# EmreAdabag/osqp

Hardware: AMD Instinct MI355X
Metric: ADMM iters/sec (single QP) (higher is better)
Workload: dtype f64; 1 GPU; config2 random sparse QP n=10000 m=20000 nnzA=200000 nnzPtriu=59985, one step = osqp_update_rho(0.1) + cold-started osqp_solve; adaptive_rho_interval=100, status=solved, graph_launches=4775, resident_gave_up=0, resident_slow_waits=0, parallelism=replicas x1 (a single QP does not shard)

## Files before the change

osqp_amd/csrc/engine.hip:

```cpp
#include <hip/hip_runtime.h>
#include <cstdio>
#include <new>
#include <cstdlib>
#include <cstring>
#include <cmath>
#include <vector>
#include <map>
#include <algorithm>
#include <mutex>
#include <condition_variable>
#include <thread>
#include <atomic>
#include <chrono>
#include "../../include/osqp_amd_engine.h"

#define TB 256
#define MAX_CHUNK 2048
#define LONG_ROW 512
#define HUGE_ROW 8192
#define MAX_PARTS 1024
#define MAX_HUGE_FOLD 4
#define INF_BOUND 1e26

#define HIPCHK(call)                                                            \
// ... 9 lines not shown
struct RowBlk { int r0, r1, k0, k1; };
#define IS_LONG(b) ((b).r1 - (b).r0 == 1 && (b).k1 - (b).k0 >= LONG_ROW)
struct __attribute__((aligned(32))) G4 { double r, w, s, m; };

struct DevMat {
  int nrows, nblk;
  int nstream;
  int nwave;
  const int    *rowptr;
  const int    *col;
  const unsigned short *col16;
  const double *val;
  const int    *split;
  const RowBlk *blk;
};

#define DENSE_MAX 128
struct DenseBlk { int c0, b, off, pitch; };
struct DenseP {
  int nblk;
  const DenseBlk *blk;
  const double *val;
};

struct State {
  int    run;
  int    done;
  int    stalled;
  int    neg_curv;
  int    iters[2];
  int    neg_curv_seen;
  int    iters_last;
  int    iters_max;
  int    iters_min;
  int    forced;
  long long iters_total;
  long long admm_done;
  double rz[2];
  double tol2;
  double gam[2], alp[2];
  int    hist_r;
  long long admm_target;
  unsigned res_epoch;
  int    res_fail;
  int    res_pipe_off;
  int    res_chk_fail;
  int    res_dbg[4];
  int    res_slow;
  int    res_slow_max;
  int    res_repub;
  int    res_slow_hist[4];
  unsigned res_slow_xcc;
  int    res_slow_last[4];
};

struct Params {
  double sigma, alpha, eps_rel, eps_abs, cinv;
  int    pcg_max_iter, use_cvec, has_scaling, pad0;
  double ex_theta;
  int    ex_h0, ex_h1;
  int    no_restart;
};

struct Ctx {
  int n, m;
  DevMat A, M;
  DevMat Mk;
  DenseP dP;
  int nh, hrow[MAX_HUGE_FOLD];
  const double *hcol;
  int gridA, gridM;
  double *xy, *z, *zt, *va, *vb, *q, *l, *u, *rho, *rhoinv, *minv, *pdiag;
  double *r, *zz, *kp, *pt0, *pt1, *dxy, *dy, *cvec;
  double *init_r, *init_z;
  double *vx, *vold;
  double *pdir, *ut;
  G4     *g4;
  int     init_stride;
  int     fin_wave_rows;
  double *vd;
  int     plain_rhs;
  const int *plain_skip;
  const unsigned short *u0map;
  double *u0pos;
  int     nelim;
  const int *erow, *ecol, *epos;
  double *rhoe, *ecoef, *edinv, *xte;
  double *D, *Dinv, *E, *Einv;
  double *part_rz, *part_rr, *part_bb, *part_pkp, *part_s0, *part_s1, *part_s2, *part_gam, *part_del;
  const double *fin_rr;
  int fin_cnt;
  double *scal;
  double *part_h;
  State  *st;
  const Params *prm;
#ifdef OSQP_AMD_TIMELINE
  unsigned long long *tl;
#endif
};

#ifdef OSQP_AMD_TIMELINE
#define TL_CAP (1 << 20)
#define TL_MARK(c, id) do { if (blockIdx.x == 0 && threadIdx.x == 0) { const unsigned long long k_ = atomicAdd((c).tl, 1ull); \
    if (k_ < TL_CAP - 2) (c).tl[1 + k_] = ((unsigned long long)(id) << 56) | (wall_clock64() & 0x00FFFFFFFFFFFFFFull); } } while (0)
#else
#define TL_MARK(c, id) do { } while (0)
#endif

enum {
  SC_PRI_U, SC_PRI_S, SC_Z_U, SC_Z_S, SC_AX_U, SC_AX_S,
  SC_DUA_U, SC_DUA_S, SC_Q_U, SC_Q_S, SC_ATY_U, SC_ATY_S, SC_PX_U, SC_PX_S,
  SC_DYN_U, SC_DYN_S, SC_DXN_U, SC_DXN_S,
  SC_ATDY_U, SC_ATDY_S, SC_PDX_U, SC_PDX_S, SC_ADX_VIOL,
  SC_OBJ, SC_DYLHS, SC_QDX,
  SC_COUNT
};
#define SCI(x) ((x) * 16)

template <int CTRL>
__device__ __forceinline__ double dpp_move(double v) {
  int lo = __double2loint(v), hi = __double2hiint(v);
  lo = __builtin_amdgcn_mov_dpp(lo, CTRL, 0xF, 0xF, true); hi = __builtin_amdgcn_mov_dpp(hi, CTRL, 0xF, 0xF, true);
  return __hiloint2double(hi, lo);
}
__device__ __forceinline__ double lane_value(double v, int lane) {
  return __hiloint2double(__builtin_amdgcn_readlane(__double2hiint(v), lane), __builtin_amdgcn_readlane(__double2loint(v), lane));
}
__device__ __forceinline__ double wave_sum(double v) {
  v += dpp_move<0xB1>(v); v += dpp_move<0x4E>(v); v += dpp_move<0x141>(v); v += dpp_move<0x140>(v);
  return (lane_value(v, 0) + lane_value(v, 16)) + (lane_value(v, 32) + lane_value(v, 48));
}

__device__ __forceinline__ double block_sum(double v, double *red) {
  v = wave_sum(v);
  const int lane = threadIdx.x & 63, w = threadIdx.x >> 6;
  __syncthreads();
  if (lane == 0) red[w] = v;
// ... 218 lines not shown
    const double rj = gone ? 0.0 : bj - prm.sigma * c.vx[j] - sA;
    const double zj = c.minv[j] * rj;
    c.init_r[(size_t)j * c.init_stride] = rj;
    c.init_z[j] = zj;
    if (c.u0pos) c.u0pos[c.u0map[j]] = zj;
    prz += rj * zj; prr += rj * rj; pbb += bj * bj;
  };
  for (int bi = blockIdx.x; bi < Mm.nstream; bi += gridDim.x) {
    const RowBlk b = Mm.blk[bi];
    stage_products<2>(Mm, b, c.vx, c.vb, lprod, lprod + MAX_CHUNK);
    __syncthreads();
    const int RL = lanes_for(b.r1 - b.r0), rg = threadIdx.x / RL, rlane = threadIdx.x % RL;
    for (int j = b.r0 + rg; j < b.r1; j += TB / RL) {
      const int a0 = Mm.rowptr[j] - b.k0, a1 = Mm.rowptr[j + 1] - b.k0;
      const double sA = row_sum_par(lprod, a0, a1, rlane, RL);
      const double sB = row_sum_par(lprod + MAX_CHUNK, a0, a1, rlane, RL);
      if (rlane == 0) row_start(j, sA, sB);
    }
    __syncthreads();
  }
  for (int bi = Mm.nstream + blockIdx.x * (TB / 64) + (threadIdx.x >> 6); bi < Mm.nblk; bi += gridDim.x * (TB / 64)) {
    const RowBlk lb = Mm.blk[bi];
    const int lane = threadIdx.x & 63;
    if (c.vd) {
      const double acc = wave_row_dot(Mm, lb.k0, lb.k1, [&](int cc) { return c.vd[cc]; });
      if (lane == 0) row_start(lb.r0, -acc, 0.0);
      continue;
    }
    double a0 = 0.0, a1 = 0.0, b0 = 0.0, b1 = 0.0;
    const bool narrow = Mm.col16 != nullptr;
    constexpr int UI = 8;
    for (int k0 = lb.k0 + lane; k0 - lane < lb.k1; k0 += 64 * UI) {
      int cc[UI]; double vv[UI], xa[UI], xb[UI];
#pragma unroll
      for (int q = 0; q < UI; ++q) {
        const int kc = min(k0 + 64 * q, lb.k1 - 1);
        cc[q] = narrow ? (int)Mm.col16[kc] : Mm.col[kc];
        vv[q] = Mm.val[kc];
      }
#pragma unroll
      for (int q = 0; q < UI; ++q) { xa[q] = c.vx[cc[q]]; xb[q] = c.vb[cc[q]]; }
#pragma unroll
      for (int q = 0; q < UI; ++q) if (k0 + 64 * q >= lb.k1) vv[q] = 0.0;
#pragma unroll
      for (int q = 0; q < UI; q += 2) { a0 += vv[q] * xa[q]; b0 += vv[q] * xb[q]; a1 += vv[q + 1] * xa[q + 1]; b1 += vv[q + 1] * xb[q + 1]; }
    }
    const double sA = wave_sum(a0 + a1), sB = wave_sum(b0 + b1);
    if (lane == 0) row_start(lb.r0, sA, sB);
  }
  block_sum3(prz, prr, pbb, red);
  if (threadIdx.x == 0) {
    c.part_rz[blockIdx.x] = prz; c.part_rr[blockIdx.x] = prr; c.part_bb[blockIdx.x] = pbb;
    if (blockIdx.x == 0) {
      st->run = 1; st->done = 0; st->neg_curv = 0; st->iters[0] = 0; st->iters[1] = 0;
      if (st->hist_r < (1 << 20)) st->hist_r += 1;
    }
  }
}

#define EPT (MAX_CHUNK / TB)

struct CgStep { double alpha, beta; bool first, stop, conv, bad; };
__device__ __forceinline__ CgStep cg_step(double rr, double gam, double del, double gam_old, double alp_old,
                                          double tol2, int iters_prev, int neg, const Params &prm, bool bench) {
  CgStep s;
  s.first = gam_old == 0.0;
  s.bad = false;
  if (s.first) { s.beta = 0.0; s.alpha = gam / del; }
  else {
    s.beta = gam / gam_old;
    const double den = del - s.beta * gam / alp_old;
    if (!(den > 0.0) && del > 0.0) {
      if (!prm.no_restart && rr <= 1e8 * tol2) { s.first = true; s.beta = 0.0; s.alpha = gam / del; }
      else { s.alpha = gam / den; s.bad = true; }
    } else s.alpha = gam / den;
  }
  if (bench) { s.beta = 0.5; s.alpha = 1e-3; s.bad = false; }
  s.conv = rr <= tol2;
  s.bad = s.bad || !(s.alpha > 0.0) || !(del > 0.0);
  s.stop = !bench && (s.conv || iters_prev >= prm.pcg_max_iter || neg || s.bad);
  return s;
}
__global__ void __launch_bounds__(TB) k_cg_A(Ctx c, int it, int flags) {
  State *st = c.st;
  TL_MARK(c, 2);
  const bool bench = flags & 4, upd_only = flags & 16, apply_only = flags & 32;
  const bool pre = (flags & 8) || apply_only;
  if (!bench && it >= (flags >> 8) && (it >= st->iters_last || st->stalled) && (!st->run || st->done)) return;
  const int stalled = st->stalled, run = st->run, done = st->done, neg = st->neg_curv;
  const int iters_prev = st->iters[(it + 1) & 1];
  const double tol2_old = st->tol2, gam_old = st->gam[(it + 1) & 1], alp_old = st->alp[(it + 1) & 1];
  const Params prm = *c.prm;
  const bool has_blk = (int)blockIdx.x < c.A.nstream;
  RowBlk b = {0, 0, 0, 0};
  if (has_blk) b = c.A.blk[blockIdx.x];
  const int cnt = b.k1 - b.k0;
  const bool small = has_blk;
  const G4 *gold = c.g4 + (size_t)((it + 1) & 1) * c.n;
  G4 *gnew = c.g4 + (size_t)(it & 1) * c.n;
  int ecol[EPT]; double eval[EPT], g0[EPT], g1[EPT], g2[EPT], g3[EPT];
  int RL = lanes_for(b.r1 - b.r0);
  int rg = threadIdx.x / RL, rlane = threadIdx.x % RL;
  int rp0 = 0, rp1 = 0;
  double prho = 0.0;
  if (small) {
    if (b.r0 + rg < b.r1) { rp0 = c.A.rowptr[b.r0 + rg]; rp1 = c.A.rowptr[b.r0 + rg + 1]; prho = c.rhoe[b.r0 + rg]; }
#pragma unroll
// ... 253 lines not shown
      const double uj = lprod[4 * DENSE_MAX + threadIdx.x], wj = (acc + sigma * uj) + hterm(jrow, false), rj = gc[jrow].r;
      gc[jrow].w = wj; pg += rj * uj; pd += wj * uj; prr += rj * rj;
    }
    __syncthreads();
  }
  block_sum3(pg, pd, prr, red);
  if (threadIdx.x == 0) { c.part_gam[blockIdx.x] = pg; c.part_del[blockIdx.x] = pd; c.part_rr[blockIdx.x] = prr; }
}


__global__ void __launch_bounds__(TB) k_huge_dot(Ctx c, const double *x, int always) {
  if (!always && !c.st->run) return;
  if (!x) {
    const State *st = c.st;
    x = (c.vx != c.va && st->iters[0] == 0 && st->iters[1] == 0) ? c.vx : c.va;
  }
  __shared__ double red[16];
  for (int bi = c.A.nwave; bi < c.A.nblk; ++bi) {
    const RowBlk hb = c.A.blk[bi];
    double s0 = 0.0, s1 = 0.0;
    int k = hb.k0 + blockIdx.x * TB + threadIdx.x;
    const int stride = gridDim.x * TB;
    for (; k + stride < hb.k1; k += 2 * stride) {
      const int c0 = c.A.col[k], c1 = c.A.col[k + stride];
      s0 += c.A.val[k] * x[c0]; s1 += c.A.val[k + stride] * x[c1];
    }
    if (k < hb.k1) s0 += c.A.val[k] * x[c.A.col[k]];
    const double tot = block_sum(s0 + s1, red);
    if (threadIdx.x == 0) c.part_h[(size_t)(bi - c.A.nwave) * gridDim.x + blockIdx.x] = tot;
  }
}
__device__ __forceinline__ double huge_row_sum(const Ctx &c, int bi, double *red) {
  const double *part = c.part_h + (size_t)(bi - c.A.nwave) * c.gridA;
  double s = 0.0;
  for (int i = threadIdx.x; i < c.gridA; i += TB) s += part[i];
  return block_sum(s, red);
}

__device__ __forceinline__ double elim_vb(const Ctx &c, const Params &prm, int i, double rho, double vbn, double x_y) {
  const int y = c.ecol[i];
  if (y < 0) return vbn;
  const double a = c.ecoef[i];
  const double by = (prm.use_cvec ? c.cvec[y] : (prm.sigma * x_y - c.q[y])) + a * vbn;
  return vbn - rho * a * by * c.edinv[i];
}

__global__ void __launch_bounds__(TB) k_admm_finalize(Ctx c) {
  State *st = c.st;
  TL_MARK(c, 4);
  if (!st->run || st->res_fail) return;
  LDS_DECL(1);
  const Params prm = *c.prm;
  double rr[1];
  reduce_parts<1>(c.fin_rr, nullptr, nullptr, c.fin_cnt, red, rr);
  const int iters = st->iters[0] > st->iters[1] ? st->iters[0] : st->iters[1];
  const bool conv = st->done == 1 || rr[0] <= st->tol2;
  const bool force = st->done == 2 || iters >= prm.pcg_max_iter || st->neg_curv;
  if (!conv && !force) {
    if (blockIdx.x == 0 && threadIdx.x == 0) st->stalled = 1;
    return;
  }
  if (blockIdx.x == 0 && threadIdx.x == 0) {
    st->stalled = 0;
    st->admm_done += 1;
    st->iters_last = iters;
    st->iters_total += iters;
    if (iters > st->iters_max) st->iters_max = iters;
    if (iters < st->iters_min) st->iters_min = iters;
    if (!conv) st->forced += 1;
    if (st->neg_curv) st->neg_curv_seen += 1;
  }
  const double alpha = prm.alpha, oma = 1.0 - prm.alpha;
  const int hist = st->hist_r;
  const double th = (hist < prm.ex_h0 ? 0.0 : (hist < prm.ex_h1 ? 0.5 : 1.0)) * prm.ex_theta;
  const bool ex = c.vx != c.va;
  const bool from_start = ex && iters == 0;
  const double *xts = from_start ? c.vx : c.va;
  double *x = c.xy, *y = c.xy + c.n;
  for (int j = blockIdx.x * TB + threadIdx.x; j < c.n; j += gridDim.x * TB) {
    if (c.nelim && c.erow[j] >= 0) continue;
    const double xo = x[j], xt = xts[j];
    const double xn = alpha * xt + oma * xo;
    c.dxy[j] = xn - xo;
    x[j] = xn;
    if (ex) { c.vx[j] = xt + th * (xt - c.vold[j]); c.vold[j] = xt; }
    if (from_start) c.va[j] = xt;
  }
  auto row_update = [&](int i, double zt) {
    const double rho = c.rho[i], rinv = c.rhoinv[i], yo = y[i], zo = c.z[i];
    const int ye = c.nelim ? c.ecol[i] : -1;
    double rz = rho * zt, xny = 0.0;
    if (ye >= 0) {
      const double a = c.ecoef[i], xoy = x[ye];
      const double by = (prm.use_cvec ? c.cvec[ye] : (prm.sigma * xoy - c.q[ye])) + a * (rho * zo - yo);
      const double xty = (by - rho * a * zt) * c.edinv[i];
      rz = c.rhoe[i] * zt;
      zt += a * xty;
      xny = alpha * xty + oma * xoy;
      c.dxy[ye] = xny - xoy; x[ye] = xny; c.xte[i] = xty;
    }
    double v = alpha * zt + oma * zo + rinv * yo;
    v = fmax(v, c.l[i]);
    const double zn = fmin(v, c.u[i]);
    const double dy = rho * (alpha * zt + oma * zo - zn);
    const double yn = yo + dy;
    c.z[i] = zn; y[i] = yn; c.dy[i] = dy; c.zt[i] = zt;
    c.va[c.n + i] = rz;
    if (ex) { c.vx[c.n + i] = rz + th * (rz - c.vold[c.n + i]); c.vold[c.n + i] = rz; }
    c.vb[c.n + i] = ye >= 0 ? elim_vb(c, prm, i, rho, rho * zn - yn, xny) : rho * zn - yn;
  };
// ... 108 lines not shown
    for (int eb = e0; eb < e1; eb += 256) {
      int j[4]; double v[4];
#pragma unroll
      for (int q = 0; q < 4; ++q) {
        const int idx = eb + q * 64 + lane;
        j[q] = -1; v[q] = 0.0;
        if (idx < e1) {
          j[q] = rc.kcj[idx];
          const int ps = rc.kps[idx];
          v[q] = (ps >= 0 ? c.M.val[ps] : 0.0) + (j[q] == i ? sigma : 0.0);
        }
      }
      for (int kc = ka; kc < kb; kc += 64) {
        const bool on = kc + lane < kb;
        const int kk = on ? c.M.col[kc + lane] - c.n : 0;
        const double ai = on ? c.M.val[kc + lane] : 0.0, rk = on ? c.rhoe[kk] : 0.0;
        const int p0 = on ? c.A.rowptr[kk] : 0, p1 = on ? c.A.rowptr[kk + 1] : 0;
        const int cnt = min(64, kb - kc);
        for (int q = 0; q < cnt; ++q) {
          const double a_i = lane_value(ai, q), r = lane_value(rk, q);
          const int s0 = lane_int(p0, q), s1 = lane_int(p1, q);
          for (int ec = s0; ec < s1; ec += 64) {
            const bool eon = ec + lane < s1;
            const int cj = eon ? c.A.col[ec + lane] : -1;
            const double av = eon ? c.A.val[ec + lane] : 0.0;
            const int len = min(64, s1 - ec);
            for (int e = 0; e < len; ++e) {
              const int cjb = lane_int(cj, e);
              const double t = r * (a_i * lane_value(av, e));
#pragma unroll
              for (int q4 = 0; q4 < 4; ++q4) if (j[q4] == cjb) v[q4] += t;
            }
          }
        }
      }
      const bool igone = c.nelim && c.erow[i] >= 0;
#pragma unroll
      for (int q = 0; q < 4; ++q) {
        const int idx = eb + q * 64 + lane;
        if (idx < e1) {
          const bool gone = c.nelim && (igone || c.erow[j[q]] >= 0);
          rc.val[rc.kdst[idx]] = gone ? (j[q] == i ? 1.0 : 0.0) : v[q];
        }
      }
    }
  }
}

template <int E>
__global__ void __launch_bounds__(RES_TB) k_pcg_resident(Ctx c, ResCtx rc) {
  extern __shared__ __attribute__((aligned(16))) double rlds[];
  State *st = c.st;
  TL_MARK(c, 5);
  if (st->stalled || !st->run || st->res_fail) return;
  double *uv = rlds;
  double *seg = uv + rc.npad;
  double *sc = seg + RES_TB + RES_MAXROWS;
  double *sval = sc + 8;
#ifdef OSQP_AMD_TIMELINE
  long long *tls = reinterpret_cast<long long *>(sval + 768);
#define RTL(k) do { if (blockIdx.x == 0 && threadIdx.x == 0 && nx >= 1 && nx <= 64) tls[(nx - 1) * 5 + (k)] = wall_clock64(); } while (0)
  long long *wtl = tls + 5 * 64;
#define WTL(k) do { if (blockIdx.x == 0 && (threadIdx.x & 63) == 0 && (nx == 8 || nx == 1)) wtl[(nx == 1 ? 40 : 0) + (k) * 8 + (threadIdx.x >> 6)] = wall_clock64(); } while (0)
  if (blockIdx.x == 0 && threadIdx.x == 0) wtl[80] = wall_clock64();
#else
#define RTL(k) do { } while (0)
#define WTL(k) do { } while (0)
#endif
  const int g = blockIdx.x, t = threadIdx.x, lane = t & 63, wv = t >> 6;
  const int nwg = rc.nwg, npad = rc.npad;
  const ResWG w = rc.wg[g];
  const Params prm = *c.prm;
  const unsigned ep0 = st->res_epoch;
  const bool sabotage = rc.inject > 0 && g == rc.nwg - 1 && st->admm_done + 1 == rc.inject;
  bool pipe = rc.pipe && !st->res_pipe_off && !prm.no_restart;
  const bool prod = wv != 0;
  const int tt = t - 64;
  double kv[E]; unsigned short kc[E];
#pragma unroll
  for (int k = 0; k < E; ++k) { kv[k] = 0.0; kc[k] = 0; }
  unsigned long long brk = 0ull;
  int slot0 = 0;
  if (prod) {
#pragma unroll
    for (int k = 0; k < E; ++k) {
      const size_t idx = ((size_t)g * E + k) * RES_PT + tt;
      kv[k] = rc.val[idx]; kc[k] = rc.col[idx];
    }
    brk = rc.brk[(size_t)g * RES_PT + tt];
    slot0 = rc.slot0[(size_t)g * RES_PT + tt];
  }
  int sr0 = 0, sr1 = 0;
  int ppos[4];
#pragma unroll
  for (int q = 0; q < 4; ++q) { const int o = lane + 64 * q; ppos[q] = 0; if (o < rc.nwg) { const ResWG wo = rc.wg[o]; ppos[q] = wo.pos + wo.nr; } }
  double rr0 = 0.0, bb = 0.0;
  for (int i = lane; i < c.gridM; i += 64) { rr0 += c.part_rr[i]; bb += c.part_bb[i]; }
  rr0 = wave_sum(rr0); bb = wave_sum(bb);
  const double tol2 = fmax(prm.eps_rel * prm.eps_rel * bb, prm.eps_abs * prm.eps_abs);
  if (rr0 <= tol2) {
    if (g == 0 && t == 0) { st->done = 1; st->tol2 = tol2; }
    return;
  }
  const bool own = wv == 0 && lane < w.nr;
  const int j = w.r0 + lane;
  double r_ = 0, u_ = 0, w_ = 0, p_ = 0, s_ = 0, x_ = 0, mi = 0, x0_ = 0, r0_ = 0;
  double z_ = 0, q_ = 0;
  if (own) {
    r_ = c.init_r[(size_t)j * c.init_stride]; u_ = c.init_z[j]; x_ = c.vx[j]; mi = c.minv[j];
    x0_ = x_; r0_ = r_;
    sr0 = rc.segrow[(size_t)g * (RES_MAXROWS + 1) + lane]; sr1 = rc.segrow[(size_t)g * (RES_MAXROWS + 1) + lane + 1];
  }
  if (t == 0) sc[3] = 0.0;
  __syncthreads();
  int nx = 0;
  unsigned tag = ep0;
  int par = 0;

  auto vec_exchange = [&](double val, bool ride) __attribute__((always_inline)) -> bool {
    double e0 = 0.0, e1 = 0.0, e2 = 0.0;
    ++nx; tag = ep0 + (unsigned)nx; par = (int)(tag & 1u);
    if (sabotage && nx == 3) return false;
    RTL(0);
    const __amdgpu_buffer_rsrc_t rs = res_rsrc(rc.ubuf + (size_t)par * npad, (size_t)npad * 8);
    if (wv == 0) {
      if (lane < w.nr) {
        u32x2 d; d.x = (unsigned)__double2loint(val); d.y = (unsigned)__double2hiint(val);
        __builtin_amdgcn_raw_buffer_store_b64(d, rs, (w.pos + lane) * 8, 0, AUX_SC1);
      }
      if (ride) { e0 = wave_sum(own ? r_ * u_ : 0.0); e1 = wave_sum(own ? w_ * u_ : 0.0); e2 = wave_sum(own ? r_ * r_ : 0.0); }
      if (lane < 3) {
        const double v = lane == 0 ? e0 : (lane == 1 ? e1 : e2);
        u32x2 d; d.x = (unsigned)__double2loint(v); d.y = (unsigned)__double2hiint(v);
        __builtin_amdgcn_raw_buffer_store_b64(d, rs, (w.pos + w.nr + lane) * 8, 0, AUX_SC1);
      }
      asm volatile("s_waitcnt vmcnt(0)" ::: "memory");
      if (lane == 0) __hip_atomic_store(rc.flags + (size_t)g * RES_FSTRIDE, tag, __ATOMIC_RELAXED, __HIP_MEMORY_SCOPE_AGENT);
    }
    if (wv < rc.npw) {
      const int o = t;
      bool pend = o < nwg && o != g;
      int miss16 = -1;
      unsigned seen = 0, rounds = 0;
      long long t0 = wall_clock64();
      int late = 0;
      bool gave = false;
      while (true) {
        if (pend) {
          seen = __hip_atomic_load(rc.flags + (size_t)o * RES_FSTRIDE, __ATOMIC_RELAXED, __HIP_MEMORY_SCOPE_AGENT);
          pend = (int)(seen - tag) < 0;
        }
        if (!__any(pend)) break;
        if (++rounds & 15u) { __builtin_amdgcn_s_sleep(1); continue; }
        const int verdict = res_spin_check(st, t0, late);
        if (verdict) {
          const unsigned long long miss = __ballot(pend);
          const int fl = miss ? (int)__ffsll((long long)miss) - 1 : 0;
          const unsigned sv = (unsigned)__builtin_amdgcn_readlane((int)seen, fl);
          if (lane == 0) { res_note(st, rc.dbg, g, verdict, 1, nx, miss ? 64 * wv + fl : -1, sv, t0, rounds, 0); sc[3] = 1.0; }
          gave = true;
          break;
        }
        if (rounds == 16u) { const unsigned long long ms = __ballot(pend); miss16 = ms ? 64 * wv + (int)__ffsll((long long)ms) - 1 : -1; }
// ... 90 lines not shown
      unsigned seen = 0, rounds = 0;
      long long t0 = wall_clock64();
      int late = 0;
      bool gave = false;
      while (true) {
        u32x2 gv[6];
#pragma unroll
        for (int q = 0; q < 6; ++q) if (pend & (1u << q)) gv[q] = __builtin_amdgcn_raw_buffer_load_b64(rg, (o * RES_GSTRIDE + q) * 8, 0, AUX_SC1 | AUX_VOL);
#pragma unroll
        for (int q = 0; q < 6; ++q)
          if (pend & (1u << q)) { if (gv[q].y == tag) { svw[q] = gv[q].x; pend &= ~(1u << q); } else seen = gv[q].y; }
        if (!__any(pend != 0)) break;
        asm volatile("" ::: "memory");
        if (++rounds & 15u) { __builtin_amdgcn_s_sleep(1); continue; }
        const int verdict = res_spin_check(st, t0, late);
        if (verdict) {
          const unsigned long long miss = __ballot(pend != 0);
          const int fl = miss ? (int)__ffsll((long long)miss) - 1 : 0;
          const unsigned sv = (unsigned)__builtin_amdgcn_readlane((int)seen, fl);
          const int gi = __builtin_amdgcn_readlane((int)pend, fl);
          if (lane == 0) { res_note(st, rc.dbg, g, verdict, 2, nx, miss ? 64 * wv + fl : -1, sv, t0, rounds, gi); sc[3] = 1.0; }
          gave = true;
          break;
        }
        if (rounds == 16u) { const unsigned long long ms = __ballot(pend != 0); miss16 = ms ? 64 * wv + (int)__ffsll((long long)ms) - 1 : -1; }
        if ((rounds & 63u) == 0 && wv == 0) {
          if (lane < 6) {
            const double v = lane < 2 ? pg : (lane < 4 ? pd : prr);
            const unsigned half = (lane & 1) ? (unsigned)__double2hiint(v) : (unsigned)__double2loint(v);
            __hip_atomic_store(gb + (size_t)g * RES_GSTRIDE + lane, ((unsigned long long)tag << 32) | half, __ATOMIC_RELAXED, __HIP_MEMORY_SCOPE_AGENT);
          }
          if (lane == 0) atomicAdd(&st->res_repub, 1);
        }
        if ((rounds & 255u) == 0) __builtin_amdgcn_fence(__ATOMIC_ACQUIRE, "agent");
        __builtin_amdgcn_s_sleep(1);
      }
      if (rounds >= 16u && lane == 0 && !gave) res_slow_note(st, t0, nx, g, miss16, 2);
    }
    __syncthreads();
    if (wv == 0) {
      double a0 = 0.0, a1 = 0.0, a2 = 0.0;
#pragma unroll
      for (int q = 0; q < 4; ++q)
        if (lane + 64 * q < nwg) { a0 += sval[3 * (lane + 64 * q)]; a1 += sval[3 * (lane + 64 * q) + 1]; a2 += sval[3 * (lane + 64 * q) + 2]; }
      a0 = wave_sum(a0); a1 = wave_sum(a1); a2 = wave_sum(a2);
      if (lane == 0) { sc[0] = a0; sc[1] = a1; sc[2] = a2; }
    }
    __syncthreads();
    RTL(4);
    return sc[3] == 0.0;
  };

  double gam_old = 0.0, alp_old = 0.0;
  int iters = 0;
  bool conv = false, bad = false, failed = false;
  int mode = pipe ? 0 : 3;
  int check_why = 0;
  int checks3 = 0;
  bool have_u0 = rc.u0_direct;
  while (true) {
    double val = u_, m_ = 0.0;
    if (mode == 1) { m_ = mi * w_; val = m_; }
    else if (mode == 2) val = x_ - x0_;
    if (have_u0) { ++nx; tag = ep0 + (unsigned)nx; par = (int)(tag & 1u); load_u0(); have_u0 = false; }
    else if (!vec_exchange(val, mode == 1)) { failed = true; break; }
    WTL(0);
    products_issue();
    WTL(1);
    CgStep cs{};
    if (mode == 1 && wv == 0) {
      double a0 = 0.0, a1 = 0.0, a2 = 0.0;
#pragma unroll
      for (int q = 0; q < 4; ++q) if (lane + 64 * q < nwg) { a0 += uv[ppos[q]]; a1 += uv[ppos[q] + 1]; a2 += uv[ppos[q] + 2]; }
      const double gam = wave_sum(a0), del = wave_sum(a1), rr = wave_sum(a2);
      cs = cg_step(rr, gam, del, gam_old, alp_old, tol2, iters, 0, prm, false);
      gam_old = gam; alp_old = cs.alpha;
      if (lane == 0) sc[4] = cs.stop ? (cs.conv ? 1.0 : 2.0) : 0.0;
    }
    WTL(2);
    const double kx = products_finish();
    WTL(3);
    if (mode == 0) { w_ = kx; mode = 1; continue; }
    if (mode == 1) {
      const double verdict = sc[4];
      if (verdict != 0.0) { check_why = verdict == 1.0 ? 0 : 1; mode = 2; continue; }
      ++iters;
      if (own) {
        z_ = cs.first ? kx : (kx + cs.beta * z_);
        q_ = cs.first ? m_ : (m_ + cs.beta * q_);
        s_ = cs.first ? w_ : (w_ + cs.beta * s_);
        p_ = cs.first ? u_ : (u_ + cs.beta * p_);
        x_ += cs.alpha * p_;
        r_ -= cs.alpha * s_;
        u_ -= cs.alpha * q_;
        w_ -= cs.alpha * z_;
      }
      WTL(4);
      if (iters >= 64) { check_why = 2; mode = 2; }
      continue;
    }
    if (mode == 2) {
      const double rt = r0_ - kx;
      if (!scal_exchange(0.0, 0.0, own ? rt * rt : 0.0)) { failed = true; break; }
      if (sc[2] <= 2.0 * tol2) { conv = true; break; }
      if (own) { r_ = rt; u_ = mi * rt; }
      gam_old = 0.0; alp_old = 0.0;
      if (check_why == 3) ++checks3;
      if (g == 0 && t == 0) { if (check_why != 2) st->res_chk_fail += 1; if (check_why < 2) st->res_pipe_off = 1; }
      __syncthreads();
      mode = 3;
      continue;
    }
    w_ = kx;
    if (!scal_exchange(own ? r_ * u_ : 0.0, own ? w_ * u_ : 0.0, own ? r_ * r_ : 0.0)) { failed = true; break; }
    const double gam = sc[0], del = sc[1], rr = sc[2];
    cs = cg_step(rr, gam, del, gam_old, alp_old, tol2, iters, 0, prm, false);
    if (cs.stop) {
      if (cs.conv && checks3 < 2) { check_why = 3; mode = 2; continue; }
      conv = cs.conv; bad = cs.bad && !cs.conv; break;
    }
    ++iters; gam_old = gam; alp_old = cs.alpha;
    if (own) {
      p_ = cs.first ? u_ : (u_ + cs.beta * p_);
      s_ = cs.first ? w_ : (w_ + cs.beta * s_);
      x_ += cs.alpha * p_;
      r_ -= cs.alpha * s_;
      u_ = mi * r_;
    }
  }
  if (failed) {
    if (t == 0) {
      __hip_atomic_store(&st->res_fail, 1, __ATOMIC_RELAXED, __HIP_MEMORY_SCOPE_AGENT);
      int *d = rc.dbg + (size_t)RES_DBG * g;
      d[0] = nx; d[1] = mode; d[2] = iters;
      if (sabotage) { d[3] = 4; d[7] = (int)__builtin_amdgcn_s_getreg((3 << 11) | 20); d[8] = (int)(unsigned)wall_clock64(); }
    }
    return;
  }
  if (own && iters > 0) c.va[j] = x_;
#ifdef OSQP_AMD_TIMELINE
  if (g == 0 && t == 0) {
    const int cnt = (nx < 64 ? nx : 64) * 5;
    const unsigned long long k0 = atomicAdd(c.tl, (unsigned long long)cnt + 1);
    if (k0 + cnt + 1 < TL_CAP - 2) {
      for (int q = 0; q < cnt; ++q) c.tl[1 + k0 + q] = ((unsigned long long)(10 + q % 5) << 56) | ((unsigned long long)tls[q] & 0x00FFFFFFFFFFFFFFull);
      c.tl[1 + k0 + cnt] = (15ull << 56) | (wall_clock64() & 0x00FFFFFFFFFFFFFFull);
    }
    if (nx >= 8) {
      const unsigned long long k1 = atomicAdd(c.tl, 80ull);
      if (k1 + 80 < TL_CAP - 2) {
        for (int q = 0; q < 40; ++q) c.tl[1 + k1 + q] = ((unsigned long long)(20 + q) << 56) | ((unsigned long long)(wtl[q] - wtl[0]) & 0x00FFFFFFFFFFFFFFull);
        for (int q = 0; q < 40; ++q) c.tl[1 + k1 + 40 + q] = ((unsigned long long)(60 + q) << 56) | ((unsigned long long)(wtl[40 + q] - wtl[80]) & 0x00FFFFFFFFFFFFFFull);
      }
    }
  }
#endif
  if (g == 0 && t == 0) {
    st->iters[0] = iters; st->iters[1] = 0;
    st->done = conv ? 1 : 2;
    if (bad) st->neg_curv = 1;
    st->tol2 = tol2;
    st->res_epoch = ep0 + (unsigned)nx;
  }
}


struct BrCtx { int nwg; const int *blk0; double *sbuf; int *dbg; };

template <int NH>
__global__ void __launch_bounds__(RES_TB) k_pcg_blockres(Ctx c, BrCtx bc) {
  constexpr int NV = 3 + NH;
  __shared__ double ul[256];
  __shared__ double red[8 * 8];
  __shared__ double tot[8];
  __shared__ double sval[256 * NV];
  State *st = c.st;
  TL_MARK(c, 6);
  if (st->stalled || !st->run || st->res_fail) return;
  const int g = blockIdx.x, t = threadIdx.x, lane = t & 63, wv = t >> 6, nwg = bc.nwg;
#ifdef OSQP_AMD_TIMELINE
  __shared__ long long btl[6 * 64];
#define BTL(k) do { if (blockIdx.x == 0 && threadIdx.x == 0 && nx >= 1 && nx <= 64) btl[(nx - 1) * 6 + (k)] = wall_clock64(); } while (0)
#else
#define BTL(k) do { } while (0)
#endif
  const Params prm = *c.prm;
  const unsigned ep0 = st->res_epoch;
  const int rl = t >> 1, h = t & 1;
  int j = -1, cb = 0, bw = 0, c0 = 0, pitch = 0; size_t off = 0;
  {
    int base = 0;
    for (int q = bc.blk0[g]; q < bc.blk0[g + 1]; ++q) {
      const DenseBlk d = c.dP.blk[q];
      if (rl >= base && rl < base + d.b) { j = d.c0 + (rl - base); cb = base; bw = d.b; c0 = d.c0; off = (size_t)d.off; pitch = d.pitch; }
      base += d.b;
    }
  }
  const bool row = j >= 0, own = row && h == 0;
  double dadd = 0.0, hc[NH > 0 ? NH : 1], hrho[NH > 0 ? NH : 1];
#pragma unroll
  for (int q = 0; q < NH; ++q) { hc[q] = 0.0; hrho[q] = c.rho[c.hrow[q]]; }
  if (row) {
    dadd = prm.sigma;
    for (int k = c.M.split[j]; k < c.M.rowptr[j + 1]; ++k) {
      const int i = c.M.col[k] - c.n;
      bool huge = false;
#pragma unroll
      for (int q = 0; q < NH; ++q) huge |= i == c.hrow[q];
      if (!huge) { const double a = c.M.val[k]; dadd += c.rho[i] * a * a; }
    }
#pragma unroll
    for (int q = 0; q < NH; ++q) hc[q] = c.hcol[(size_t)q * c.n + j];
// ... 1321 lines not shown
        }
    }
    int nseg = 0, next_row = 0;
    for (int t = 0; t < RES_PT; t++) {
      slot0[(size_t)g * RES_PT + t] = (unsigned short)nseg;
      unsigned long long b = 0;
      for (int k = 0; k < E; k++) {
        if (t * E + k >= w.cnt) break;
        const int le = ord[t * E + k];
        const size_t sl = ((size_t)g * E + k) * RES_PT + t;
        col[sl] = rowpos[Kcol[base + le]]; rowl[sl] = (unsigned char)rowof[le]; kdst[base + le] = (int)sl;
        while (next_row <= rowof[le]) segrow[(size_t)g * (RES_MAXROWS + 1) + next_row++] = (unsigned short)nseg;
        const bool last = k == E - 1 || t * E + k + 1 >= w.cnt || rowof[ord[t * E + k + 1]] != rowof[le];
        if (last) { b |= 1ull << k; nseg++; }
      }
      brk[(size_t)g * RES_PT + t] = b;
    }
    for (int r = next_row; r <= RES_MAXROWS; r++) segrow[(size_t)g * (RES_MAXROWS + 1) + r] = (unsigned short)nseg;
    if (nseg > RES_TB + RES_MAXROWS) seg_over = 1;
  }
  });
  if (seg_over.load()) return 0;
  const auto tb2 = std::chrono::steady_clock::now();
  if (po) {
    po->ok = true; po->nwg = nwg; po->E = E; po->npad = npad; po->nnzK = nnzK;
    po->wg = wg; po->Kptr = Kptr; po->Kcol = Kcol; po->kdst = kdst; po->rowpos = rowpos; po->col = col; po->brk = brk;
    return 0;
  }
  ResCtx rc{};
  rc.nwg = nwg; rc.E = E; rc.npad = npad;
  rc.npw = (nwg + 63) / 64;
  rc.pipe = 1;
  if (const char *x = getenv("OSQP_AMD_RESIDENT_PIPE")) rc.pipe = atoi(x) != 0;
  rc.u0_direct = 1;
  rc.inject = 0;
  if (const char *x = getenv("OSQP_AMD_RESIDENT_INJECT")) rc.inject = atoi(x);
  if (const char *x = getenv("OSQP_AMD_RESIDENT_U0")) rc.u0_direct = atoi(x) != 0;
  unsigned short *d_rowpos = nullptr;
  ResWG *d_wg = nullptr; unsigned short *d_col = nullptr, *d_slot0 = nullptr, *d_segrow = nullptr; unsigned char *d_rowl = nullptr;
  int *d_krp = nullptr, *d_kcj = nullptr, *d_kps = nullptr, *d_kdst = nullptr; unsigned long long *d_brk = nullptr;
  if (dev_alloc(e, &d_wg, wg.size()) || dev_alloc(e, &rc.val, slots) || dev_alloc(e, &d_col, slots) || dev_alloc(e, &d_rowl, slots) ||
      dev_alloc(e, &d_krp, Kptr.size()) || dev_alloc(e, &d_kcj, Kcol.size()) || dev_alloc(e, &d_kps, Kps.size()) || dev_alloc(e, &d_kdst, kdst.size()) ||
      dev_alloc(e, &d_brk, brk.size()) || dev_alloc(e, &d_slot0, slot0.size()) ||
      dev_alloc(e, &d_segrow, segrow.size()) || dev_alloc(e, &d_rowpos, rowpos.size()) || dev_alloc(e, &rc.ubuf, (size_t)2 * rc.npad) ||
      dev_alloc_polled(e, &rc.flags, (size_t)nwg * RES_FSTRIDE) || dev_alloc(e, &rc.dbg, (size_t)nwg * RES_DBG) || dev_alloc_polled(e, &rc.sbuf, (size_t)2 * nwg * RES_GSTRIDE)) return HIPENG_ERR_HIP;
#define UP(dst, src) HIPCHK(hipMemcpyAsync(dst, (src).data(), (src).size() * sizeof((src)[0]), hipMemcpyHostToDevice, e->stream))
  UP(d_wg, wg); UP(d_rowpos, rowpos); UP(d_col, col); UP(d_rowl, rowl); UP(d_krp, Kptr); UP(d_kcj, Kcol); UP(d_kps, Kps); UP(d_kdst, kdst); UP(d_brk, brk); UP(d_slot0, slot0); UP(d_segrow, segrow);
#undef UP
  HIPCHK(hipStreamSynchronize(e->stream));
  {
    double *d_u0pos = nullptr;
    if (dev_alloc(e, &d_u0pos, (size_t)rc.npad)) return HIPENG_ERR_HIP;
    e->c.u0map = d_rowpos; e->c.u0pos = d_u0pos;
  }
  rc.wg = d_wg; rc.rowpos = d_rowpos; rc.col = d_col; rc.rowl = d_rowl; rc.krp = d_krp; rc.kcj = d_kcj; rc.kps = d_kps; rc.kdst = d_kdst; rc.brk = d_brk; rc.slot0 = d_slot0; rc.segrow = d_segrow;
  e->rc = rc;
  e->res_lds = ((size_t)rc.npad + RES_TB + RES_MAXROWS + 3 + 16 + 768 + 5 * 64 + 96) * sizeof(double);
  int rcode = 0;
  switch (E) {
    case 8: rcode = res_set_lds<8>(e->res_lds); break;   case 16: rcode = res_set_lds<16>(e->res_lds); break;
    case 20: rcode = res_set_lds<20>(e->res_lds); break; case 24: rcode = res_set_lds<24>(e->res_lds); break;
    case 32: rcode = res_set_lds<32>(e->res_lds); break; case 48: rcode = res_set_lds<48>(e->res_lds); break;
    default: rcode = res_set_lds<64>(e->res_lds); break;
  }
  if (rcode) RES_NO("the launch's LDS request was refused");
  e->res_nnz = nnzK;
  e->res_on = e->res_use = true;
  if (e->trace) {
    const auto tb3 = std::chrono::steady_clock::now();
    auto ms = [](std::chrono::steady_clock::time_point a, std::chrono::steady_clock::time_point b) { return std::chrono::duration<double, std::milli>(b - a).count(); };
    fprintf(stderr, "[osqp_amd] resident PCG: nnz(K)=%lld, %d workgroups x %d threads x %d entries, %zu B LDS; host: pattern %.0f ms, layout %.0f ms, upload %.0f ms\n",
            nnzK, nwg, RES_TB, E, e->res_lds, ms(tb0, tb1), ms(tb1, tb2), ms(tb2, tb3));
  }
  return 0;
}


static bool blocks_eligible(hipeng *e) {
  if (e->dP_blks.empty()) return false;
  int next = 0;
  for (const DenseBlk &d : e->dP_blks) { if (d.c0 != next || d.b > DENSE_MAX) return false; next += d.b; }
  if (next != e->n) return false;
  if ((int)e->A.blk.size() - e->A.nwave != (int)e->hrows.size()) return false;
  std::vector<char> ishuge(std::max(1, e->m), 0);
  for (int hr : e->hrows) ishuge[hr] = 1;
  for (int i = 0; i < e->m; i++) if (!ishuge[i] && e->A.rowptr[i + 1] - e->A.rowptr[i] != 1) return false;
  return true;
}
static bool blocks_coupled_eligible(hipeng *e, std::vector<int> &rows) {
  if (e->dP_blks.empty()) return false;
  int next = 0;
  for (const DenseBlk &d : e->dP_blks) { if (d.c0 != next || d.b > DENSE_MAX) return false; next += d.b; }
  if (next != e->n) return false;
  int cap = CPL_MAX;
  if (const char *x = getenv("OSQP_AMD_BLOCK_COUPLED_MAX")) cap = std::max(0, std::min(CPL_MAX, atoi(x)));
  rows.clear();
  for (int i = 0; i < e->m; i++) if (e->A.rowptr[i + 1] - e->A.rowptr[i] >= 2) { if ((int)rows.size() >= cap) return false; rows.push_back(i); }
  return !rows.empty();
}
static int build_blockdirect(hipeng *e) {
  int want = 1;
  if (const char *x = getenv("OSQP_AMD_RESIDENT")) want = atoi(x);
  if (const char *x = getenv("OSQP_AMD_RESIDENT_BLOCKS")) want = want && atoi(x);
  if (const char *x = getenv("OSQP_AMD_BLOCK_DIRECT")) want = want && atoi(x);
  if (!want) return 0;
  std::vector<int> crows;
// ... 660 lines not shown
  return 0;
}

static int next_K(int want, int cap) {
  int K = 2;
  while (K < want) K = (K < 32) ? K + 2 : (K < 96 ? K + 4 : ((K + K / 4 + 1) & ~1));
  if (K > cap) K = std::max(2, (cap + 1) & ~1);
  return K;
}

static int resident_gave_up(hipeng *e, const State &s, bool quiet) {
  const int nwg = e->res_kind == 2 ? e->bc.nwg : e->rc.nwg;
  int *ddbg = e->res_kind == 2 ? e->bc.dbg : e->rc.dbg;
  std::vector<int> d((size_t)nwg * RES_DBG, 0);
  bool have = ddbg && hipMemcpy(d.data(), ddbg, d.size() * sizeof(int), hipMemcpyDeviceToHost) == hipSuccess;
  const bool injected = have && e->res_kind == 1 && e->rc.inject > 0 && d[(size_t)RES_DBG * (nwg - 1) + 3] == 4;
  if (!quiet || !injected) {
    fprintf(stderr, "osqp_amd: a resident PCG launch gave up waiting for its workgroups%s; %s with the launch-per-step kernels "
                    "[wait %d (1 flags, 2 granules) of exchange %d: workgroup %d missed workgroup %d]\n",
            injected ? " (injected by OSQP_AMD_RESIDENT_INJECT)" : " (GPU shared with another stream or process?)",
            e->res_fails >= 2 ? "continuing for good" : "finishing this call", s.res_dbg[0], s.res_dbg[1], s.res_dbg[2], s.res_dbg[3]);
    if (have) {
      std::map<long long, int> hist;
      for (int g = 0; g < nwg; g++) hist[((long long)d[(size_t)RES_DBG * g] << 16) | ((d[(size_t)RES_DBG * g + 1] & 255) << 8) | (d[(size_t)RES_DBG * g + 3] & 255)]++;
      fprintf(stderr, "osqp_amd:   workgroups by (exchange, mode, how they left: 1/2 own flag/granule wait timed out, 3 saw the give-up word, 4 injected, 0 never waited):");
      for (auto &h : hist) fprintf(stderr, " (%lld, %lld, %lld) x %d;", h.first >> 16, (h.first >> 8) & 255, h.first & 255, h.second);
      fprintf(stderr, " epoch base %u\n", s.res_epoch);
      const int wg = s.res_dbg[2], ow = s.res_dbg[3];
      if (wg >= 0 && wg < nwg) {
        const int *w = &d[(size_t)RES_DBG * wg];
        fprintf(stderr, "osqp_amd:   waiter %d (XCC %d): waited %.1f us, %d rounds, last read 0x%08x from workgroup %d (expected tag 0x%08x), gave up at clock 0x%08x\n",
                wg, w[7], w[6] * 0.01, w[9], (unsigned)w[5], w[4], s.res_epoch + (unsigned)w[0], (unsigned)w[8]);
        if (ow >= 0 && ow < nwg) {
          const int *o = &d[(size_t)RES_DBG * ow];
          unsigned long long memword = 0; bool got = false;
          if (s.res_dbg[0] == 1 && e->res_kind == 1) { unsigned f = 0; got = hipMemcpy(&f, e->rc.flags + (size_t)ow * RES_FSTRIDE, 4, hipMemcpyDeviceToHost) == hipSuccess; memword = f; }
          else {
            const double *sb = e->res_kind == 2 ? e->bc.sbuf : e->rc.sbuf;
            const unsigned tag = s.res_epoch + (unsigned)w[0];
            int gi = 0; while (gi < 15 && !((w[10] >> gi) & 1)) gi++;
            got = hipMemcpy(&memword, reinterpret_cast<const unsigned long long *>(sb) + ((size_t)(tag & 1u) * nwg + ow) * RES_GSTRIDE + gi, 8, hipMemcpyDeviceToHost) == hipSuccess;
            memword >>= 32;
          }
          fprintf(stderr, "osqp_amd:   owner %d (XCC %d): stood in exchange %d (left: %d), published at clock 0x%08x (its give-up 0x%08x minus %.1f us of its own wait); "
                          "the word in memory now: %s0x%08llx\n", ow, o[7], o[0], o[3], (unsigned)(o[8] - o[6]), (unsigned)o[8], o[6] * 0.01, got ? "" : "(unreadable) ", memword);
        }
      }
    }
  }
  e->res_use = false;
  e->res_fails += 1;
  e->res_gave_up += 1;
  HIPCHK(hipMemsetAsync(&e->c.st->res_fail, 0, sizeof(int), e->stream));
  e->h_state->res_epoch = s.res_epoch + (1u << 20);
  HIPCHK(hipMemcpyAsync(&e->c.st->res_epoch, &e->h_state->res_epoch, sizeof(unsigned), hipMemcpyHostToDevice, e->stream));
  HIPCHK(hipStreamSynchronize(e->stream));
  HIPCHK(hipMemsetAsync(e->c.st->res_dbg, 0, sizeof(int) * 4, e->stream));
  if (ddbg) HIPCHK(hipMemsetAsync(ddbg, 0, d.size() * sizeof(int), e->stream));
  return 0;
}

extern "C" int hipeng_run_admm(hipeng *e, c_int count) {
  if (!e || count < 0) return HIPENG_ERR_ARG;
  HIPCHK(hipSetDevice(e->device));
  State s;
  if (e->trace >= 2) {
    if (const char *mp = getenv("OSQP_AMD_TRACE_MAPS")) {
      static bool dumped = false;
      if (!dumped) {
        dumped = true;
        if (FILE *in = fopen("/proc/self/maps", "r")) {
          if (FILE *out = fopen(mp, "w")) { char buf[4096]; size_t k; while ((k = fread(buf, 1, sizeof buf, in)) > 0) fwrite(buf, 1, k, out); fclose(out); }
          fclose(in);
        }
      }
    }
  }
  if (count == 0) return 0;
  if (e->elim_rhs_dirty) {
    if (e->c.nelim && e->m > 0) hipLaunchKernelGGL(k_refresh_m, dim3(elem_grid(e->m)), dim3(TB), 0, e->stream, e->c, 0);
    e->elim_rhs_dirty = false;
  }
  if (e->res_on && !e->res_use && e->res_fails < 3) e->res_use = true;
  bool had_fail = false;
  const long long start = e->admm_total, target = start + (long long)count;
  *e->h_target = target;
  HIPCHK(hipMemcpyAsync(&e->c.st->admm_target, e->h_target, sizeof(long long), hipMemcpyHostToDevice, e->stream));
  HIPCHK(hipMemsetAsync(&e->c.st->iters_max, 0, sizeof(int), e->stream));
  HIPCHK(hipMemsetAsync(&e->c.st->iters_min, 0x7f, sizeof(int), e->stream));
  if (e->start_dirty) { if (reset_start(e)) return HIPENG_ERR_HIP; e->start_dirty = false; }
  long long remaining = count;
  const int cap = std::max(2, e->prm.pcg_max_iter);
  static const int khead = getenv("OSQP_AMD_KHEAD") ? atoi(getenv("OSQP_AMD_KHEAD")) : 1;
  int guard = 0, call_max = 0;
  s.admm_done = start; s.iters_last = 0; s.iters_total = 0; s.forced = 0; s.neg_curv_seen = 0;
  static const int segs = getenv("OSQP_AMD_GRAPH_SEGS") ? std::max(1, std::min(32, atoi(getenv("OSQP_AMD_GRAPH_SEGS")))) : 5;
  while (remaining > 0) {
    const bool resident = e->res_use;
    CuLease lease;
    if (resident && e->res_kind < 3) lease.take(e->device, e->res_cus, e->res_kind == 2 ? e->bc.nwg : e->rc.nwg);
    const long long burst = std::min<long long>(remaining, (e->calibrated || resident) ? 128 : 2);
    TR2(e, "launch burst=%lld K=%d", burst, e->K);
    const int R = (resident || e->K <= 48) ? segs : 1;
    const int gK = resident ? 0 : e->K, gS = resident ? 0 : e->spec_lo;
    hipGraphExec_t gR = nullptr, g1 = nullptr;
    if (burst >= R && R > 1 && get_graph(e, gK, R, gS, &gR)) return HIPENG_ERR_HIP;
// ... 349 lines not shown
```

Baseline: 7806 ADMM iters/s.

## Defer resident PCG true-residual check to finalize kernel with continuation

Instead of performing the true-residual check (mode 2) inside the resident PCG kernel with an extra grid-wide scalar exchange, the kernel now writes x, the residual and per-workgroup partial norms to global memory and exits with done=3. The finalize kernel reduces the partials and either accepts convergence or marks the step stalled, and a relaunched resident kernel then continues PCG from the saved state. This removes one cross-workgroup synchronisation from the resident loop. In exchange, a failed check now costs a kernel relaunch plus state reload, and the continuation logic adds new state fields and extra complexity.

After: 7769 ADMM iters/s. Within noise of the previous version (-0.5%).

```diff
diff --git a/osqp_amd/csrc/engine.hip b/osqp_amd/csrc/engine.hip
--- a/osqp_amd/csrc/engine.hip
+++ b/osqp_amd/csrc/engine.hip
@@ -85,6 +85,8 @@
   int    res_slow_hist[4];
   unsigned res_slow_xcc;
   int    res_slow_last[4];
+  int    res_why;
+  int    res_checks3;
 };
 
 struct Params {
@@ -116,6 +118,8 @@
   const int *plain_skip;
   const unsigned short *u0map;
   double *u0pos;
+  double *res_part, *res_rt;
+  int     res_nparts;
   int     nelim;
   const int *erow, *ecol, *epos;
   double *rhoe, *ecoef, *edinv, *xte;
@@ -440,7 +444,7 @@
   if (threadIdx.x == 0) {
     c.part_rz[blockIdx.x] = prz; c.part_rr[blockIdx.x] = prr; c.part_bb[blockIdx.x] = pbb;
     if (blockIdx.x == 0) {
-      st->run = 1; st->done = 0; st->neg_curv = 0; st->iters[0] = 0; st->iters[1] = 0;
+      st->run = 1; st->done = 0; st->neg_curv = 0; st->iters[0] = 0; st->iters[1] = 0; st->res_checks3 = 0;
       if (st->hist_r < (1 << 20)) st->hist_r += 1;
     }
   }
@@ -800,10 +804,34 @@
   LDS_DECL(1);
   const Params prm = *c.prm;
   double rr[1];
-  reduce_parts<1>(c.fin_rr, nullptr, nullptr, c.fin_cnt, red, rr);
+  const int done = st->done;
+  bool conv;
+  if (done == 3) {
+    if (threadIdx.x < 64) {
+      double a = 0.0;
+      for (int q = threadIdx.x; q < c.res_nparts; q += 64) a += c.res_part[q];
+      a = wave_sum(a);
+      if (threadIdx.x == 0) red[0] = a;
+    }
+    __syncthreads();
+    conv = red[0] <= 2.0 * st->tol2;
+    if (!conv) {
+      if (blockIdx.x == 0 && threadIdx.x == 0) {
+        const int why = st->res_why;
+        st->stalled = 1;
+        if (why != 2) st->res_chk_fail += 1;
+        if (why < 2) st->res_pipe_off = 1;
+        if (why == 3) st->res_checks3 += 1;
+      }
+      return;
+    }
+    __syncthreads();
+  } else {
+    reduce_parts<1>(c.fin_rr, nullptr, nullptr, c.fin_cnt, red, rr);
+    conv = done == 1 || rr[0] <= st->tol2;
+  }
   const int iters = st->iters[0] > st->iters[1] ? st->iters[0] : st->iters[1];
-  const bool conv = st->done == 1 || rr[0] <= st->tol2;
-  const bool force = st->done == 2 || iters >= prm.pcg_max_iter || st->neg_curv;
+  const bool force = done == 2 || iters >= prm.pcg_max_iter || st->neg_curv;
   if (!conv && !force) {
     if (blockIdx.x == 0 && threadIdx.x == 0) st->stalled = 1;
     return;
@@ -1018,7 +1046,8 @@
   extern __shared__ __attribute__((aligned(16))) double rlds[];
   State *st = c.st;
   TL_MARK(c, 5);
-  if (st->stalled || !st->run || st->res_fail) return;
+  if (!st->run || st->res_fail) return;
+  const bool cont = st->stalled != 0;
   double *uv = rlds;
   double *seg = uv + rc.npad;
   double *sc = seg + RES_TB + RES_MAXROWS;
@@ -1039,7 +1068,8 @@
   const Params prm = *c.prm;
   const unsigned ep0 = st->res_epoch;
   const bool sabotage = rc.inject > 0 && g == rc.nwg - 1 && st->admm_done + 1 == rc.inject;
-  bool pipe = rc.pipe && !st->res_pipe_off && !prm.no_restart;
+  bool pipe = rc.pipe && !st->res_pipe_off && !prm.no_restart && !cont;
+  const int iters_before = cont ? st->iters[0] : 0, checks_before = cont ? st->res_checks3 : 0;
   const bool prod = wv != 0;
   const int tt = t - 64;
   double kv[E]; unsigned short kc[E];
@@ -1064,7 +1094,7 @@
   for (int i = lane; i < c.gridM; i += 64) { rr0 += c.part_rr[i]; bb += c.part_bb[i]; }
   rr0 = wave_sum(rr0); bb = wave_sum(bb);
   const double tol2 = fmax(prm.eps_rel * prm.eps_rel * bb, prm.eps_abs * prm.eps_abs);
-  if (rr0 <= tol2) {
+  if (rr0 <= tol2 && !cont) {
     if (g == 0 && t == 0) { st->done = 1; st->tol2 = tol2; }
     return;
   }
@@ -1075,6 +1105,10 @@
   if (own) {
     r_ = c.init_r[(size_t)j * c.init_stride]; u_ = c.init_z[j]; x_ = c.vx[j]; mi = c.minv[j];
     x0_ = x_; r0_ = r_;
+    if (cont) {
+      r_ = c.res_rt[j]; u_ = mi * r_; x_ = c.va[j];
+      if (c.vx == c.va) { x0_ = c.res_rt[c.n + j]; }
+    }
     sr0 = rc.segrow[(size_t)g * (RES_MAXROWS + 1) + lane]; sr1 = rc.segrow[(size_t)g * (RES_MAXROWS + 1) + lane + 1];
   }
   if (t == 0) sc[3] = 0.0;
@@ -1271,12 +1305,12 @@
   };
 
   double gam_old = 0.0, alp_old = 0.0;
-  int iters = 0;
-  bool conv = false, bad = false, failed = false;
+  int iters = iters_before;
+  bool conv = false, bad = false, failed = false, deferred = false;
   int mode = pipe ? 0 : 3;
   int check_why = 0;
-  int checks3 = 0;
-  bool have_u0 = rc.u0_direct;
+  const int checks3 = checks_before;
+  bool have_u0 = rc.u0_direct && !cont;
   while (true) {
     double val = u_, m_ = 0.0;
     if (mode == 1) { m_ = mi * w_; val = m_; }
@@ -1320,15 +1354,14 @@
     }
     if (mode == 2) {
       const double rt = r0_ - kx;
-      if (!scal_exchange(0.0, 0.0, own ? rt * rt : 0.0)) { failed = true; break; }
-      if (sc[2] <= 2.0 * tol2) { conv = true; break; }
-      if (own) { r_ = rt; u_ = mi * rt; }
-      gam_old = 0.0; alp_old = 0.0;
-      if (check_why == 3) ++checks3;
-      if (g == 0 && t == 0) { if (check_why != 2) st->res_chk_fail += 1; if (check_why < 2) st->res_pipe_off = 1; }
-      __syncthreads();
-      mode = 3;
-      continue;
+      if (wv == 0) {
+        if (own) { c.va[j] = x_; c.res_rt[j] = rt; if (c.vx == c.va) c.res_rt[c.n + j] = x0_; }
+        const double prr = wave_sum(own ? rt * rt : 0.0);
+        if (lane == 0) c.res_part[g] = prr;
+      }
+      RTL(4);
+      deferred = true;
+      break;
     }
     w_ = kx;
     if (!scal_exchange(own ? r_ * u_ : 0.0, own ? w_ * u_ : 0.0, own ? r_ * r_ : 0.0)) { failed = true; break; }
@@ -1356,7 +1389,7 @@
     }
     return;
   }
-  if (own && iters > 0) c.va[j] = x_;
+  if (own && iters > 0 && !deferred) c.va[j] = x_;
 #ifdef OSQP_AMD_TIMELINE
   if (g == 0 && t == 0) {
     const int cnt = (nx < 64 ? nx : 64) * 5;
@@ -1376,7 +1409,8 @@
 #endif
   if (g == 0 && t == 0) {
     st->iters[0] = iters; st->iters[1] = 0;
-    st->done = conv ? 1 : 2;
+    st->done = deferred ? 3 : (conv ? 1 : 2);
+    if (deferred) st->res_why = check_why;
     if (bad) st->neg_curv = 1;
     st->tol2 = tol2;
     st->res_epoch = ep0 + (unsigned)nx;
@@ -2804,6 +2838,8 @@
     double *d_u0pos = nullptr;
     if (dev_alloc(e, &d_u0pos, (size_t)rc.npad)) return HIPENG_ERR_HIP;
     e->c.u0map = d_rowpos; e->c.u0pos = d_u0pos;
+    if (dev_alloc(e, &e->c.res_part, (size_t)nwg) || dev_alloc(e, &e->c.res_rt, (size_t)2 * e->n)) return HIPENG_ERR_HIP;
+    e->c.res_nparts = nwg;
   }
   rc.wg = d_wg; rc.rowpos = d_rowpos; rc.col = d_col; rc.rowl = d_rowl; rc.krp = d_krp; rc.kcj = d_kcj; rc.kps = d_kps; rc.kdst = d_kdst; rc.brk = d_brk; rc.slot0 = d_slot0; rc.segrow = d_segrow;
   e->rc = rc;
@@ -3570,6 +3606,7 @@
   e->res_fails += 1;
   e->res_gave_up += 1;
   HIPCHK(hipMemsetAsync(&e->c.st->res_fail, 0, sizeof(int), e->stream));
+  HIPCHK(hipMemsetAsync(&e->c.st->stalled, 0, sizeof(int), e->stream));
   e->h_state->res_epoch = s.res_epoch + (1u << 20);
   HIPCHK(hipMemcpyAsync(&e->c.st->res_epoch, &e->h_state->res_epoch, sizeof(unsigned), hipMemcpyHostToDevice, e->stream));
   HIPCHK(hipStreamSynchronize(e->stream));
```
